# lisqzqng/Video-based-gait-analysis-for-dementia

Measured on AMD Instinct MI355X. Metric: frames/sec (224x224, seq=16), higher is better.
Workload: dtype f32

## Files before the change

video-based-gait-analysis-for-dementia_amd/csrc/grnet_run.cpp:

```cpp
#include "grnet_impl.h"

namespace grk { thread_local GraphRecorder* g_recorder = nullptr; }

int grnet::allocate() {
    if (plan_arena(compact, arena_plan)) return fail(GRNET_ESTATE, "the activation arena could not be planned: a launch group or the assignment violates the sharing rule");
    const size_t total = (size_t)arena_plan.total;
    arena_floats = total;
    void* q = nullptr;
    if (hipMalloc(&q, total * sizeof(float)) != hipSuccess)
        return fail(GRNET_ENOMEM, std::string("hipMalloc of the ") + (compact ? "compact " : "") + "activation arena (" + std::to_string(total * 4 >> 20) + " MiB) failed");
    arena = static_cast<float*>(q);
    if (hipMemset(arena, 0, 64 * sizeof(float)) != hipSuccess) return fail(GRNET_EHIP, "hipMemset failed");
    zeros = arena;
    if (hipEventCreateWithFlags(&ev_fork, hipEventDisableTiming) != hipSuccess) return fail(GRNET_EHIP, "hipEventCreate failed");
    if (int rc = install_schedule(max_frames)) return rc;
    if (hipStreamCreateWithFlags(&capture_stream, hipStreamNonBlocking) != hipSuccess) return fail(GRNET_EHIP, "hipStreamCreate failed");
    const size_t n = max_frames;
    int rc;
    if ((rc = dev_alloc(&d_plf, n * 128 * 24))) return rc;
    if ((rc = dev_alloc(&d_csf, n * 64 * 24))) return rc;
    if ((rc = dev_alloc(&d_stats, softmax_pool_ws_floats((int)n)))) return rc;
    if ((rc = dev_alloc(&d_rot6d, n * 144))) return rc;
    if ((rc = dev_alloc(&d_shape, n * 10))) return rc;
    if ((rc = dev_alloc(&d_cam, n * 3))) return rc;
// ... 291 lines not shown
    for (size_t oi = 0; oi < ops.size(); ++oi) {
        const Op& op = ops[oi];
        s = lane_stream[op.lane];
        const int lane = multi_lane ? op.lane : 0;
        if (lanes)
            for (int w : op.waits) HIP_TRY(hipStreamWaitEvent(s, op_events[w], 0));
        if (convs_only && op.kind != Op::CONV && op.kind != Op::FUSEUP) {
            if (lanes && op.record) HIP_TRY(hipEventRecord(op_events[oi], s));
            continue;
        }
        if (tl_start && !rec) HIP_TRY(hipEventRecord((*tl_start)[oi], s));
        if (rec) {
            rec->deps.clear();
            rec->n_chain = lane_last[lane] ? 1 : 0;
            if (lane_last[lane]) rec->deps.push_back(lane_last[lane]);
            if (multi_lane)
                for (int w : op.waits)
                    if (op_node[w] && std::find(rec->deps.begin(), rec->deps.end(), op_node[w]) == rec->deps.end()) rec->deps.push_back(op_node[w]);
        }
        static const char* abl_skip = GRNET_AB_STR(ABL_SKIP);
        if (abl_skip && (op.kind == Op::CONV || op.kind == Op::FUSEUP)) {
            const std::string lbl = op_label(op);
            bool skip = false;
            for (const char* q = abl_skip; *q;) {
                const char* e = strchr(q, ',');
                const std::string pat = e ? std::string(q, e) : std::string(q);
                if (!pat.empty() && lbl.find(pat) != std::string::npos) skip = true;
                q = e ? e + 1 : q + strlen(q);
            }
            if (skip) {
                if (tl_end && !rec) HIP_TRY(hipEventRecord((*tl_end)[oi], s));
                if (lanes && op.record) HIP_TRY(hipEventRecord(op_events[oi], s));
                continue;
            }
        }
        switch (op.kind) {
            case Op::CONVERT:
                HIP_TRY(launch_nchw_f32_to_nhwc_bf16(frames, base(v_in8), n, 3, 224, 224, 8, s));
                ++launches;
                break;
            case Op::CONV: {
                int nl = 1;
                if (int rc = launch_conv_op(convs[op.conv_idx], frames, n, s, &nl)) return rc;
                launches += nl;
                break;
            }
            case Op::SUM: {
                const auto& sv = sum_views[op.conv_idx];
                SumArgs a = op.sum;
                a.N = n;
                bind(sv.out, a.out, a.out_ctot, a.out_coff);
                for (int k = 0; k < a.n_add; ++k) {
                    bind(sv.adds[k].v, a.add[k], a.add_ctot[k], a.add_coff[k]);
                    a.add_shift[k] = sv.adds[k].shift;
                }
                if (dtype == 1) HIP_TRY(launch_fuse_sum_bf16(a, s));
                else HIP_TRY(launch_fuse_sum(a, s));
                ++launches;
                break;
            }
            case Op::FUSEUP:
                if (int rc = launch_fuse_up_op(fuse_ups[op.conv_idx], n, s)) return rc;
                ++launches;
                break;
            case Op::BILINEAR:
                if (dtype == 1) HIP_TRY(launch_bilinear2x_bf16(base(op.bin), base(op.bout), n, op.bin.c, op.bin.h, op.bin.w, s));
                else HIP_TRY(launch_bilinear2x(base(op.bin), base(op.bout), n, op.bin.c, op.bin.h, op.bin.w, s));
                ++launches;
                break;
            case Op::POOL:
                if (dtype == 1)
                    HIP_TRY(launch_softmax_pool_bf16(base(v_heat), v_heat.ctot, bf16_at(v_smpl_feats), 128, v_smpl_feats.ctot, bf16_at(v_csmap), 64,
                                                     v_csmap.ctot, d_stats, n, 56 * 56, s));
                else
                    HIP_TRY(launch_softmax_pool(base(v_heat), 25, base(v_smpl_feats), 128, base(v_csmap), 64, plf, csf, d_stats, n, 56 * 56, s));
                ++launches;
                break;
            case Op::TAIL:
                HIP_TRY(launch_head_tail(d_stats, true, plf, csf, tailw, rot6d, d_shape, d_cam, rotmat, theta, n, s));
                ++launches;
                break;
            case Op::SMPL:
                HIP_TRY(launch_smpl(d_shape, rotmat, d_cam, smpl, d_A, verts, kp3d, kp2d, n, s));
                launches += 4;
                break;
        }
        if (tl_end && !rec) HIP_TRY(hipEventRecord((*tl_end)[oi], s));
        if (lanes && op.record) HIP_TRY(hipEventRecord(op_events[oi], s));
        if (rec && !rec->deps.empty()) lane_last[lane] = op_node[oi] = rec->deps[0];
    }
    s = caller;
    if (lanes)
        for (int l = 1; l < lanes_used; ++l) {
            if (!join_lane[l]) continue;
            HIP_TRY(hipEventRecord(ev_join[l], side[l]));
            HIP_TRY(hipStreamWaitEvent(s, ev_join[l], 0));
        }
    if (!convs_only) {
        auto copy_out = [&](float* dst, const float* src, size_t bytes) -> int {
            if (!dst) return 0;
            if (!rec) { HIP_TRY(hipMemcpyAsync(dst, src, bytes, hipMemcpyDeviceToDevice, s)); return 0; }
            std::vector<hipGraphNode_t> deps;
            for (hipGraphNode_t nd : lane_last) if (nd) deps.push_back(nd);
            hipGraphNode_t node = nullptr;
            HIP_TRY(hipGraphAddMemcpyNode1D(&node, rec->graph, deps.data(), deps.size(), dst, src, bytes, hipMemcpyDeviceToDevice));
            return 0;
        };
        int rc;
        if (dtype == 1) {
            auto conv_out = [&](float* dst, const View& v) -> int {
                if (!dst) return 0;
                if (rec) {
                    rec->deps.clear();
                    for (hipGraphNode_t nd : lane_last) if (nd) rec->deps.push_back(nd);
                }
                HIP_TRY(launch_nhwc_bf16_to_nchw_f32(base(v), dst, n, v.c, v.h, v.w, v.ctot, v.coff, s));
                return 0;
            };
            if ((rc = conv_out(o.features, v_cat))) return rc;
            if ((rc = conv_out(o.part_attn, v_heat))) return rc;
            if ((rc = conv_out(o.smpl_feats, v_smpl_feats))) return rc;
        } else {
        if ((rc = copy_out(o.features, base(v_cat), (size_t)n * 480 * 3136 * 4))) return rc;
        if ((rc = copy_out(o.part_attn, base(v_heat), (size_t)n * 25 * 3136 * 4))) return rc;
        if ((rc = copy_out(o.smpl_feats, base(v_smpl_feats), (size_t)n * 128 * 3136 * 4))) return rc;
        }
        launches_last = launches;
    }
    return 0;
}

int grnet::head_from_feats(const float* plf, const float* csf, int n, const grnet_outputs_t& o, hipStream_t s) {
    const auto [rot6d, rotmat, theta, verts, kp3d, kp2d] = head_outputs(o);
    HIP_TRY(launch_head_tail_from_feats(plf, csf, tailw, rot6d, d_shape, d_cam, rotmat, theta, n, s));
    HIP_TRY(launch_smpl(d_shape, rotmat, d_cam, smpl, d_A, verts, kp3d, kp2d, n, s));
    if (o.point_local_feat && o.point_local_feat != plf) HIP_TRY(hipMemcpyAsync(o.point_local_feat, plf, (size_t)n * 3072 * 4, hipMemcpyDeviceToDevice, s));
    if (o.cam_shape_feats && o.cam_shape_feats != csf) HIP_TRY(hipMemcpyAsync(o.cam_shape_feats, csf, (size_t)n * 1536 * 4, hipMemcpyDeviceToDevice, s));
    return 0;
}

int grnet::gait_correct(const float* plf, const float* csf, const float* cam, int cam_ld, const float* bbox, const float* cimg, int b, int T,
                        const grnet_outputs_t& o, const grnet_gait_outputs_t& g, hipStream_t s) {
    if (int rc = gru_fault_check()) return rc;
    const size_t M = (size_t)b * T;
    const bool taps = taps_armed;
    if (taps) {
        size_t need = 0;
        if (featcorr_tap_floats(b, T, &need) != hipSuccess) { taps_armed = false; return fail(GRNET_EHIP, "device query for the tap layout failed"); }
        if (int rc = taps_begin(need + gru_tap_floats(b, T), "a gait-correction call")) return rc;
    }
    const size_t gru_need = gru_ws_floats(M, b);
    auto al = [](size_t f) { return (f + 63) & ~(size_t)63; };
    const size_t own = al(M * 3) + al((size_t)b * 3) + al(M * 4) + al(M * 3072);
    float* ws = nullptr;
    if (int rc = temporal_scratch(kGemmWsFloats + gru_need + featcorr_ws_floats(b, T) + own, &ws)) return rc;
    GemmWorkspaceLease lease(ws, kGemmWsFloats);
    float* p = ws + kGemmWsFloats;
    float* cparams = g.pred_cparam ? g.pred_cparam : p;   p += al(M * 3);
    float* avg = g.pred_avg ? g.pred_avg : p;             p += al((size_t)b * 3);
    float* phase = g.pred_phase ? g.pred_phase : p;       p += al(M * 4);
    float* new_plf = g.point_local_feat ? g.point_local_feat : p;   p += al(M * 3072);
    float* xc_buf = nullptr;
    const GruWorkspace w = gru_carve(p, M, b, &xc_buf);
    float* fws = p + gru_need;
    {
        TapLease tap_lease(taps ? &tap_sink : nullptr);
        HIP_TRY(launch_gait_cparams(cam, cam_ld, bbox, cimg, cparams, (int)M, s));
// ... 248 lines not shown
```

video-based-gait-analysis-for-dementia_amd/csrc/head_kernels.hip:

```cpp
#include "kernels.h"
#include "device.h"

namespace grk {

__global__ __launch_bounds__(256) void fuse_sum_kernel(const SumArgs a) {
    const int HW = a.H * a.W, n = blockIdx.x / a.C, c = blockIdx.x - n * a.C;
    const float inv_w = 1.0f / (float)a.W;
    for (int pix = threadIdx.x * 4; pix < HW; pix += 1024) {
        f32x4 v = f32x4{0.f, 0.f, 0.f, 0.f};
        for (int k = 0; k < a.n_add; ++k) {
            const int sh = a.add_shift[k];
            if (sh == 0) {
                v += *reinterpret_cast<const f32x4*>(a.add[k] + ((size_t)n * a.add_ctot[k] + a.add_coff[k] + c) * HW + pix);
            } else {
                const int hs = a.H >> sh, ws = a.W >> sh;
                const float* ap = a.add[k] + ((size_t)n * a.add_ctot[k] + a.add_coff[k] + c) * (hs * ws);
#pragma unroll
                for (int r = 0; r < 4; ++r) {
                    const int y = (int)(((float)(pix + r) + 0.5f) * inv_w), x = (pix + r) - y * a.W;
                    v[r] += ap[(y >> sh) * ws + (x >> sh)];
                }
            }
        }
        if (a.relu) {
// ... 398 lines not shown
            const f32x4 wv = *reinterpret_cast<const f32x4*>(wr + 4 * k), x = *reinterpret_cast<const f32x4*>(cs + 4 * k);
            acc += x * wv;
        }
        s_sp[o][seg] = (acc[0] + acc[1]) + (acc[2] + acc[3]);
    }
    __syncthreads();
    if (tid < 144) {
        const float acc = (s_pp[0][tid] + s_pp[1][tid]) + (s_pp[2][tid] + s_pp[3][tid]);
        s_pose[tid] = acc;
        rot6d[(size_t)n * 144 + tid] = acc;
    } else if (tid < 157) {
        const int o = tid - 144;
        float acc = 0.f;
#pragma unroll
        for (int seg = 0; seg < 8; ++seg) acc += s_sp[o][seg];
        s_sc[o] = acc + (o < 10 ? w.shape_b[o] : w.cam_b[o - 10]);
    }
    __syncthreads();
    if (tid < 24) {
        float R[9], aa[3];
        rot6d_to_rotmat_dev(&s_pose[tid * 6], R);
#pragma unroll
        for (int k = 0; k < 9; ++k) rotmat[(size_t)n * 216 + tid * 9 + k] = R[k];
        rotmat_to_aa_dev(R, aa);
        theta[(size_t)n * 85 + 3 + tid * 3 + 0] = aa[0];
        theta[(size_t)n * 85 + 3 + tid * 3 + 1] = aa[1];
        theta[(size_t)n * 85 + 3 + tid * 3 + 2] = aa[2];
    }
    if (tid >= 64 && tid < 74) {
        const int o = tid - 64;
        shape[(size_t)n * 10 + o] = s_sc[o];
        theta[(size_t)n * 85 + 75 + o] = s_sc[o];
    }
    if (tid >= 128 && tid < 131) {
        const int o = tid - 128;
        cam[(size_t)n * 3 + o] = s_sc[10 + o];
        theta[(size_t)n * 85 + o] = s_sc[10 + o];
    }
}

hipError_t launch_head_tail(const float* pool_ws, bool range_stats, float* plf, float* csf, TailWeights w, float* rot6d, float* shape, float* cam,
                            float* rotmat, float* theta, int N, hipStream_t s) {
    GRK_TRY(launch_k(head_tail_kernel<true>, dim3(N), dim3(256), 0, s, pool_ws + (size_t)N * kPoolStatsFloats, range_stats ? pool_ws : (const float*)nullptr, plf, csf,
                     w, rot6d, shape, cam, rotmat, theta));
    return hipGetLastError();
}

hipError_t launch_head_tail_from_feats(const float* plf, const float* csf, TailWeights w, float* rot6d, float* shape, float* cam, float* rotmat,
                                       float* theta, int N, hipStream_t s) {
    GRK_TRY(launch_k(head_tail_kernel<false>, dim3(N), dim3(256), 0, s, (const float*)nullptr, (const float*)nullptr, const_cast<float*>(plf), const_cast<float*>(csf), w,
                     rot6d, shape, cam, rotmat, theta));
    return hipGetLastError();
}

__global__ __launch_bounds__(256) void rot6d_to_rotmat_kernel(const float* __restrict__ x, float* __restrict__ R, int m) {
    const int i = blockIdx.x * 256 + threadIdx.x;
    if (i >= m) return;
    float xi[6], r[9];
#pragma unroll
    for (int k = 0; k < 6; ++k) xi[k] = x[(size_t)i * 6 + k];
    rot6d_to_rotmat_dev(xi, r);
#pragma unroll
    for (int k = 0; k < 9; ++k) R[(size_t)i * 9 + k] = r[k];
}
__global__ __launch_bounds__(256) void rotmat_to_aa_kernel(const float* __restrict__ R, float* __restrict__ aa, int m) {
    const int i = blockIdx.x * 256 + threadIdx.x;
    if (i >= m) return;
    float r[9], a[3];
#pragma unroll
    for (int k = 0; k < 9; ++k) r[k] = R[(size_t)i * 9 + k];
    rotmat_to_aa_dev(r, a);
#pragma unroll
    for (int k = 0; k < 3; ++k) aa[(size_t)i * 3 + k] = a[k];
}
hipError_t launch_rot6d_to_rotmat(const float* x, float* R, int m, hipStream_t s) {
    GRK_TRY(launch_k(rot6d_to_rotmat_kernel, dim3((m + 255) / 256), dim3(256), 0, s, x, R, m));
    return hipGetLastError();
}
hipError_t launch_rotmat_to_aa(const float* R, float* aa, int m, hipStream_t s) {
    GRK_TRY(launch_k(rotmat_to_aa_kernel, dim3((m + 255) / 256), dim3(256), 0, s, R, aa, m));
    return hipGetLastError();
}

__global__ __launch_bounds__(320) void smpl_chain_kernel(const float* __restrict__ betas, const float* __restrict__ rotmat, SmplTables t,
                                                           float* __restrict__ A_ws, float* __restrict__ kp3d, float* __restrict__ feat) {
    __shared__ float J[24][3];
    __shared__ float G[24][12];
    __shared__ float Rs[216];
    __shared__ int par[24], depth[24];
    const int n = blockIdx.x, tid = threadIdx.x;
    for (int e = tid; e < 216; e += 320) Rs[e] = rotmat[(size_t)n * 216 + e];
    if (tid < 24) par[tid] = t.parents[tid];
    for (int e = tid; e < 72; e += 320) {
        float v = t.J_template[e];
#pragma unroll
        for (int l = 0; l < 10; ++l) v += t.J_shapedirs[e * 10 + l] * betas[(size_t)n * 10 + l];
        J[e / 3][e % 3] = v;
    }
    for (int e = tid; e < kBlendK; e += 320) {
        float v = 0.f;
        if (e < 207) v = rotmat[(size_t)n * 216 + 9 + e] - ((e % 9 == 0 || e % 9 == 4 || e % 9 == 8) ? 1.f : 0.f);
        else if (e < 217) v = betas[(size_t)n * 10 + e - 207];
        else if (e == 217) v = 1.f;
        feat[(size_t)n * kBlendK + e] = v;
    }
    __syncthreads();
    if (tid < 24) {
        int d = 0;
        for (int p = par[tid]; p >= 0 && d < 24; p = par[p]) ++d;
        depth[tid] = d;
    }
    __syncthreads();
    const int ji = tid / 12, rc = tid - ji * 12, r = rc >> 2, c = rc & 3;
    const bool mine = tid < 288;
    const int myd = mine ? depth[ji] : -1, p = mine ? par[ji] : 0;
    for (int d = 0; d < 24; ++d) {
        if (mine && myd == d) {
            if (d == 0) {
                G[ji][rc] = c < 3 ? Rs[ji * 9 + r * 3 + c] : J[ji][r];
            } else {
                const float g0 = G[p][r * 4 + 0], g1 = G[p][r * 4 + 1], g2 = G[p][r * 4 + 2];
                if (c < 3) {
                    const float* Ri = Rs + ji * 9;
                    G[ji][rc] = g0 * Ri[c] + g1 * Ri[3 + c] + g2 * Ri[6 + c];
                } else {
                    const float t0 = J[ji][0] - J[p][0], t1 = J[ji][1] - J[p][1], t2 = J[ji][2] - J[p][2];
                    G[ji][rc] = g0 * t0 + g1 * t1 + g2 * t2 + G[p][r * 4 + 3];
                }
            }
        }
        __syncthreads();
        if (d >= 1 && __syncthreads_count(mine && myd > d) == 0) break;
    }
    for (int e = tid; e < 24 * 12; e += 320) {
        const int i = e / 12, rc2 = e % 12, r2 = rc2 / 4, c2 = rc2 % 4;
        float v = G[i][rc2];
        if (c2 == 3) {
            kp3d[((size_t)n * 29 + i) * 3 + r2] = v;
            v -= G[i][r2 * 4 + 0] * J[i][0] + G[i][r2 * 4 + 1] * J[i][1] + G[i][r2 * 4 + 2] * J[i][2];
        }
        A_ws[(size_t)n * 288 + e] = v;
    }
}

constexpr int kNumVerts = 6890;
constexpr int kBlendCols = kNumVerts * 3;

template <int MT>
__device__ __forceinline__ void blend_pass(const float* __restrict__ As, const float (&bv)[kBlendK / 4], float* __restrict__ Cs, int l15, int lq, int wave) {
    constexpr int LD = kBlendK + 1, KS = kBlendK / 4;
    f32x4 acc[MT];
#pragma unroll
    for (int m = 0; m < MT; ++m) acc[m] = f32x4{0.f, 0.f, 0.f, 0.f};
    const float* a0 = As + l15 * LD + lq;
#pragma unroll
    for (int ks = 0; ks < KS; ++ks)
#pragma unroll
        for (int m = 0; m < MT; ++m) acc[m] = __builtin_amdgcn_mfma_f32_16x16x4f32(a0[m * 16 * LD + 4 * ks], bv[ks], acc[m], 0, 0, 0);
#pragma unroll
    for (int m = 0; m < MT; ++m)
#pragma unroll
        for (int r = 0; r < 4; ++r) Cs[(m * 16 + lq * 4 + r) * 64 + wave * 16 + l15] = acc[m][r];
}

__global__ __launch_bounds__(256, 2) void smpl_blend_mfma_kernel(const float* __restrict__ feat, const float* __restrict__ blend, float* __restrict__ vposed,
                                                               int N) {
    constexpr int LD = kBlendK + 1, KS = kBlendK / 4;
    __shared__ float As[64 * LD];
    __shared__ __align__(16) float Cs[64 * 64];
    const int tid = threadIdx.x, lane = tid & 63, wave = tid >> 6, l15 = lane & 15, lq = lane >> 4;
    const int col = blockIdx.x * 64 + wave * 16 + l15;
    const bool cok = col < kBlendCols;
    const float* bp = blend + (cok ? col : 0) + (size_t)lq * kBlendCols;
    float bv[KS];
#pragma unroll
    for (int ks = 0; ks < KS; ++ks) bv[ks] = bp[(size_t)(4 * ks) * kBlendCols];
    for (int f0 = 0; f0 < N; f0 += 64) {
        const int nf = min(64, N - f0), mtiles = (nf + 15) >> 4;
        __syncthreads();
        {
            constexpr int UPR = kBlendK / 4, NU = (64 * UPR + 255) / 256;
            f32x4 v[NU];
#pragma unroll
            for (int i = 0; i < NU; ++i) {
                const int u = tid + 256 * i, f = u / UPR;
                v[i] = (u < mtiles * 16 * UPR && f < nf) ? *reinterpret_cast<const f32x4*>(feat + (size_t)(f0 + f) * kBlendK + 4 * (u - f * UPR))
                                                           : f32x4{0.f, 0.f, 0.f, 0.f};
            }
#pragma unroll
            for (int i = 0; i < NU; ++i) {
                const int u = tid + 256 * i, f = u / UPR, k = 4 * (u - f * UPR);
                if (u < mtiles * 16 * UPR) {
                    As[f * LD + k] = v[i][0]; As[f * LD + k + 1] = v[i][1]; As[f * LD + k + 2] = v[i][2]; As[f * LD + k + 3] = v[i][3];
                }
            }
        }
        __syncthreads();
        switch (mtiles) {
            case 1: blend_pass<1>(As, bv, Cs, l15, lq, wave); break;
            case 2: blend_pass<2>(As, bv, Cs, l15, lq, wave); break;
            case 3: blend_pass<3>(As, bv, Cs, l15, lq, wave); break;
            default: blend_pass<4>(As, bv, Cs, l15, lq, wave); break;
        }
        __syncthreads();
        const int cbase = blockIdx.x * 64;
#pragma unroll
        for (int i = 0; i < 8; ++i) {
            const int row = (tid >> 5) + 8 * i, c2 = (tid & 31) * 2;
            if (row < nf && cbase + c2 < kBlendCols)
                *reinterpret_cast<f32x2*>(vposed + (size_t)(f0 + row) * kBlendCols + cbase + c2) = *reinterpret_cast<const f32x2*>(Cs + row * 64 + c2);
        }
    }
}

__global__ __launch_bounds__(256) void smpl_skin_kernel(SmplTables t, const float* __restrict__ A_ws, float* __restrict__ verts) {
    __shared__ float sA[288];
    const int n = blockIdx.y, tid = threadIdx.x;
    for (int e = tid; e < 288; e += 256) sA[e] = A_ws[(size_t)n * 288 + e];
    __syncthreads();
    const int v = blockIdx.x * 256 + tid;
    if (v >= kNumVerts) return;
    float* pv = verts + ((size_t)n * kNumVerts + v) * 3;
    const float p0 = pv[0], p1 = pv[1], p2 = pv[2];
    float T[12];
#pragma unroll
    for (int e = 0; e < 12; ++e) T[e] = 0.f;
    for (int k = 0; k < t.skin_k; ++k) {
        const int j = t.skin_idx[(size_t)v * t.skin_k + k];
        const float wj = t.skin_w[(size_t)v * t.skin_k + k];
        if (j < 0) break;
#pragma unroll
        for (int e = 0; e < 12; ++e) T[e] += wj * sA[j * 12 + e];
    }
#pragma unroll
    for (int r = 0; r < 3; ++r) pv[r] = T[r * 4 + 0] * p0 + T[r * 4 + 1] * p1 + T[r * 4 + 2] * p2 + T[r * 4 + 3];
}

__global__ __launch_bounds__(256) void smpl_joints_kernel(const float* __restrict__ verts, const float* __restrict__ cam, SmplTables t,
                                                            float* __restrict__ kp3d, float* __restrict__ kp2d) {
    __shared__ float red[4][3];
    __shared__ float sj[29][3];
    const int n = blockIdx.x, tid = threadIdx.x, lane = tid & 63, wave = tid >> 6;
    const float* vn = verts + (size_t)n * kNumVerts * 3;
    float a0 = 0.f, a1 = 0.f, a2 = 0.f;
    for (int k = tid; k < t.thorax_n; k += 256) {
        const int v = t.thorax_idx[k];
        const float w = t.thorax_w[k];
        a0 += w * vn[v * 3]; a1 += w * vn[v * 3 + 1]; a2 += w * vn[v * 3 + 2];
    }
    a0 = wave_sum(a0); a1 = wave_sum(a1); a2 = wave_sum(a2);
    if (lane == 0) { red[wave][0] = a0; red[wave][1] = a1; red[wave][2] = a2; }
    if (tid < 72) sj[tid / 3][tid % 3] = kp3d[(size_t)n * 87 + tid];
    if (tid >= 96 && tid < 108) {
        const int e = tid - 96, jj = e / 3, d = e % 3;
        const int vid = jj == 0 ? 2746 : jj == 1 ? 2445 : jj == 2 ? 6191 : 5905;
        sj[24 + jj][d] = vn[vid * 3 + d];
    }
    __syncthreads();
    if (tid < 3) sj[28][tid] = red[0][tid] + red[1][tid] + red[2][tid] + red[3][tid];
    __syncthreads();
    if (tid < 87) kp3d[(size_t)n * 87 + tid] = sj[tid / 3][tid % 3];
    if (tid < 29 && cam != nullptr && kp2d != nullptr) {
        const float s = cam[(size_t)n * 3], tx = cam[(size_t)n * 3 + 1], ty = cam[(size_t)n * 3 + 2];
        const float tz = 2.f * 5000.f / (224.f * s + 1e-9f);
        const float X = sj[tid][0] + tx, Y = sj[tid][1] + ty, Z = sj[tid][2] + tz;
        kp2d[((size_t)n * 29 + tid) * 2 + 0] = 5000.f * (X / Z) / 112.f;
        kp2d[((size_t)n * 29 + tid) * 2 + 1] = 5000.f * (Y / Z) / 112.f;
    }
}

hipError_t launch_smpl(const float* betas, const float* rotmat, const float* cam, SmplTables t, float* A_ws, float* verts,
                       float* kp3d, float* kp2d, int N, hipStream_t s) {
    float* feat = A_ws + (size_t)N * 288;
    GRK_TRY(launch_k(smpl_chain_kernel, dim3(N), dim3(320), 0, s, betas, rotmat, t, A_ws, kp3d, feat));
    GRK_TRY(launch_k(smpl_blend_mfma_kernel, dim3((kBlendCols + 63) / 64), dim3(256), 0, s, (const float*)feat, t.blend, verts, N));
    GRK_TRY(launch_k(smpl_skin_kernel, dim3((kNumVerts + 255) / 256, N), dim3(256), 0, s, t, (const float*)A_ws, verts));
    GRK_TRY(launch_k(smpl_joints_kernel, dim3(N), dim3(256), 0, s, verts, cam, t, kp3d, kp2d));
    return hipGetLastError();
}

}
```

video-based-gait-analysis-for-dementia_amd/csrc/kernels.h:

```cpp
#pragma once
#include <hip/hip_runtime.h>
#include <stdint.h>
#include "raster_lines.h"
#include "seq_args.h"

#include <initializer_list>
#include <mutex>
#include <string>
#include <tuple>
#include <utility>
#include <vector>

#ifdef GRNET_ABLATION
#include <cstdlib>
#define GRNET_AB(name, dflt) (getenv("GRNET_" #name) ? atoi(getenv("GRNET_" #name)) : (dflt))
#define GRNET_AB_F(name, dflt) (getenv("GRNET_" #name) ? atof(getenv("GRNET_" #name)) : (dflt))
#define GRNET_AB_SET(name) (getenv("GRNET_" #name) != nullptr)
#define GRNET_AB_STR(name) getenv("GRNET_" #name)
#else
#define GRNET_AB(name, dflt) (dflt)
#define GRNET_AB_F(name, dflt) (dflt)
#define GRNET_AB_SET(name) false
#define GRNET_AB_STR(name) (static_cast<const char*>(nullptr))
#endif
// ... 113 lines not shown
    int pw_stream;
    int dbg;
    int prio;
    int blk0, wsplit;
};

hipError_t launch_conv(ConvArgs a, hipStream_t s, int tile_hint = 0);
struct ConvChoice { int family = 0, tps = 0, tcs = 0, nw = 0, waves = 0, width_variant = 0, rows = 0; };
hipError_t conv_choose(const ConvArgs& a, int tile_hint, ConvChoice* out);
int conv_pick_tc(int Cout);
hipError_t conv_init();
const char* conv_dominant_kernel_name();

bool conv_wino4_eligible(int cin, int cout, int ks, int stride, int h, int w, int n_add);
hipError_t launch_conv_wino4(ConvArgs a, hipStream_t s, int* n_launches = nullptr);
void pack_wino4_weights(const double* w_folded , int cout, int cin, int cin_pad, int cout_pad, float* out, int map_width = 56);
int conv_wino4_blocks(int cout, int map_width);
int conv_wino4_wide(int cout, int map_width);
struct Wino4Form { int waves = 0, nb = 0, npw = 0, gx = 0, gy = 0, xcd = 0, split = 0, full = 0, rest = 0; };
hipError_t conv_wino4_form(const ConvArgs& a, Wino4Form* f);

void wino4_transform_filter(const double* g33, double* u36);
bool conv_pw_eligible(int cin, int cout, int ks, int stride, int h, int w, int n_add);
hipError_t launch_conv_pw(ConvArgs a, hipStream_t s);
bool conv_stem_eligible(int cin, int cout, int ks, int stride, int h, int w, int n_add);
hipError_t launch_conv_stem(ConvArgs a, hipStream_t s);
void pack_stem_weights(const double* w_folded , float* out );
bool conv_wino4s_eligible(int cin, int cout, int ks, int stride, int h, int w, int n_add);
hipError_t launch_conv_wino4s(ConvArgs a, hipStream_t s, int ksplit);
int conv_wino4s_images_per_tile(int map_width);
int conv_wino4s_row_tiles(int map_width, int n_images, int* last_tile_images);
void pack_wino4r_weights(const double* w_folded , int cout, int cin, float* out );
struct SumArgs {
    float* out; int out_ctot, out_coff;
    int N, C, H, W, relu, n_add;
    const float* add[4]; int add_ctot[4], add_coff[4], add_shift[4];
};
hipError_t launch_fuse_sum(const SumArgs& a, hipStream_t s);

struct FuseUpSrc { const float* x; int ctot, coff; const float* w; };
struct FuseUpOut {
    float* out; int out_ctot, out_coff;
    const float* base; int base_ctot, base_coff;
    const float* bias;
    int relu, n_extra;
    const float* extra[2]; int extra_ctot[2], extra_coff[2];
    FuseUpSrc src[3];
};
struct FuseUpArgs { int N, nb; FuseUpOut o[3]; int only = -1; };
hipError_t launch_hr_fuse_up(const FuseUpArgs& a, hipStream_t s);
void pack_fuse_up_weights(const double* w_folded , int cout, int cin, float* out );
hipError_t launch_hr_fuse_up_bf16(const FuseUpArgs& a, hipStream_t s);
void pack_fuse_up_weights_bf16(const double* w_folded , int cout, int cin, unsigned short* out );

hipError_t launch_bilinear2x(const float* in, float* out, int N, int C, int H, int W, hipStream_t s);

hipError_t launch_crop_normalise(const unsigned char* img, int H, int W, int per_image, const float* bbox, float scale, int bgr,
                                 float* out, int N, hipStream_t s);

hipError_t launch_crop_normalise_cv(const unsigned char* img, int H, int W, int per_image, const double* maps, int mstride, int bgr, float* out, int N,
                                    hipStream_t s);

hipError_t launch_softmax_pool(const float* heat, int heat_ctot, const float* featA, int CA, const float* featB, int CB,
                               float* outA, float* outB, float* prob_ws, int N, int P, hipStream_t s);

struct TailWeights {
    const float* pose_w;
    const float* shape_w;
    const float* shape_b;
    const float* cam_w;
    const float* cam_b;
};
hipError_t launch_head_tail(const float* pool_ws, bool range_stats , float* plf, float* csf, TailWeights w, float* rot6d, float* shape, float* cam,
                            float* rotmat, float* theta, int N, hipStream_t s);
hipError_t launch_head_tail_from_feats(const float* plf, const float* csf, TailWeights w, float* rot6d, float* shape, float* cam, float* rotmat,
                                       float* theta, int N, hipStream_t s);
hipError_t launch_rot6d_to_rotmat(const float* x, float* R, int m, hipStream_t s);
hipError_t launch_rotmat_to_aa(const float* R, float* aa, int m, hipStream_t s);
size_t softmax_pool_ws_floats(int N);
constexpr int kPoolStatsFloats = 7 * 24 * 2;
constexpr int kPoolSplit = 7;

constexpr int kBlendK = 220;
constexpr int kSmplWsFloatsPerFrame = 288 + kBlendK;
struct SmplTables {
    const float* blend;
    const int* skin_idx;
    const float* skin_w;
    int skin_k;
    const float* J_template;
    const float* J_shapedirs;
    const float* lbs_weights;
    const int* thorax_idx;
    const float* thorax_w;
    int thorax_n;
    const int* parents;
    int extra_ptr[10];
    const int* extra_idx;
    const float* extra_w;
};
hipError_t launch_smpl(const float* betas, const float* rotmat, const float* cam, SmplTables t, float* A_ws,
                       float* verts, float* kp3d, float* kp2d, int N, hipStream_t s);

constexpr int kOneEuroBlock = 32;
struct OneEuroCoef { float a_d, one_minus_a_d, two_pi, min_cutoff, beta; };
hipError_t launch_one_euro(const float* x, int ld, int T, OneEuroCoef c, float* xhat, hipStream_t s);
hipError_t launch_aa_to_rotmat(const float* aa, float* R, int m, const float* betas0, float* betas_out, int nb, hipStream_t s);
int smooth_joint_count(int kind);
hipError_t launch_smpl_joints54(const float* kp29, const float* verts, SmplTables t, int kind, float* joints, int n, hipStream_t s);

constexpr int kBboxMaxJoints = 64;
constexpr int kBboxMaxFrames = 4096;
constexpr double kBboxMinPixel = 500., kBboxSmallScale = 1.8;
constexpr int kMedoidRows = 256;
constexpr int kMedoidTile = 1024;
constexpr int kMedoidMaxSplits = 64;
constexpr int kMedoidBatch = 128;
struct MedoidBatch { int n; int off[kMedoidBatch + 1]; };
__host__ __device__ inline int medoid_split_columns(int n, int splits) { return ((n + splits - 1) / splits + 7) & ~7; }
hipError_t launch_bbox_prepare(const double* joints, int K, int frames, double threshold, float* points, double* hgt, hipStream_t s);
hipError_t launch_medoid_rowsum(const float* points, const MedoidBatch& b, int splits, double* partial, hipStream_t s);
hipError_t launch_medoid_argmin(const float* points, const MedoidBatch& b, int seq0, int splits, const double* partial, int* index, double* cost,
                                float* centre, hipStream_t s);
hipError_t launch_bbox_assemble(const double* hgt, const MedoidBatch& b, int seq0, int K, const float* centre, double* bbox, hipStream_t s);

constexpr int kMetricMaxJoints = 64;
constexpr int kMetricBatch = 128;
struct MetricBatch { int n; int off[kMetricBatch + 1]; };
struct MetricJoints { int n_select, n_root; unsigned char select[kMetricMaxJoints], root[kMetricMaxJoints]; };
hipError_t launch_metric_joints(const float* pred, const float* gt, int J, int frames, const MetricJoints& mj, double unit, int has_verts, double* per_frame,
                                double* transform, hipStream_t s);
hipError_t launch_metric_accel(const float* pred, const float* gt, int J, const MetricBatch& b, const MetricJoints& mj, double unit, double* per_frame,
                               hipStream_t s);
hipError_t launch_metric_verts(const float* pred, const float* gt, int V, int frames, double unit, double* per_frame, hipStream_t s);
hipError_t launch_metric_seq_means(const double* per_frame, const MetricBatch& b, int seq0, int has_verts, double* seq_sum, long long* seq_cnt,
                                   double* per_seq, hipStream_t s);
hipError_t launch_metric_total(const double* seq_sum, const long long* seq_cnt, int n_seq, double* total, hipStream_t s);
hipError_t launch_procrustes(const double* K, int k, double* R, double* sigma, hipStream_t s);

constexpr int kTransMaxPairs = 64;
constexpr int kTransBatch = 64;
struct TransPairs { int n; int p3[kTransMaxPairs], p2[kTransMaxPairs]; };
struct TransBatch { int n; int off[kTransBatch + 1]; double cam[kTransBatch][3]; };
hipError_t launch_translation_fit(const float* joints3d, const float* joints2d, int K3, int K2, const TransPairs& pairs, const TransBatch& b, double threshold,
                                  int min_joints, double* per_frame, hipStream_t s);
hipError_t launch_translation_seq(const float* joints3d, int K3, int root, const TransBatch& b, int seq0, int fill, double* per_frame, double* per_seq,
                                  hipStream_t s);

constexpr int kTrackMaxJoints = 64;
constexpr int kTrackMaxKernel = 31;
constexpr double kTrackMaxSigma = 16.;
constexpr int kTrackMaxRadius = 64;
constexpr int kTrackMaxSeqs = 8192;
constexpr int kTrackThreads = 1024;
constexpr int kTrackLdsFrames = 1024;
hipError_t launch_track_frames(const double* joints, int K, int frames, double vis_thresh, double* params, unsigned long long* words, hipStream_t s);
hipError_t launch_track_sequences(const int* off, int n_seq, const double* weights, int radius, int ksize, int pad, const double* params,
                                  const unsigned long long* words, double* work, double* boxes, int* status, int* range, hipStream_t s);
hipError_t launch_track_filter(const int* off, int n_seq, const double* x, const double* weights, int radius, int ksize, int pad, double* out, hipStream_t s);
hipError_t launch_seq_gauss_columns(const int* off, int n_seq, int channels, const double* weights, int radius, int frames, const double* raw, double* out,
                                    int cols, int col0, hipStream_t s);

constexpr int kGaitMaxWindow = 32;
constexpr int kGaitThreads = 256;
constexpr int kGaitLdsWords = 64;
struct GaitTable { int j[8]; };
inline size_t gait_mask_words(int frames, int n_seq) { return (size_t)(frames >> 6) + (size_t)n_seq + 1; }
// ... 231 lines not shown
```

Baseline: 4572.

## Fuse SMPL pipeline into two kernels: blend+chain and skin+joints

The four SMPL launches become two. The kinematic chain now runs as extra blocks inside the blend kernel, reusing its LDS, and the blend kernel stages its features directly from rotmat and betas instead of reading a feat buffer. Skinning and joint regression are merged, with the joint blocks recomputing the skinned thorax and extra vertices from vposed rather than reading finished verts. This removes two launches and the inter-kernel dependencies, at the cost of redundant skinning work in the joint block and a larger per-frame workspace.

```diff
diff --git a/video-based-gait-analysis-for-dementia_amd/csrc/grnet_run.cpp b/video-based-gait-analysis-for-dementia_amd/csrc/grnet_run.cpp
--- a/video-based-gait-analysis-for-dementia_amd/csrc/grnet_run.cpp
+++ b/video-based-gait-analysis-for-dementia_amd/csrc/grnet_run.cpp
@@ -397,7 +397,7 @@
                 break;
             case Op::SMPL:
                 HIP_TRY(launch_smpl(d_shape, rotmat, d_cam, smpl, d_A, verts, kp3d, kp2d, n, s));
-                launches += 4;
+                launches += 2;
                 break;
         }
         if (tl_end && !rec) HIP_TRY(hipEventRecord((*tl_end)[oi], s));
diff --git a/video-based-gait-analysis-for-dementia_amd/csrc/head_kernels.hip b/video-based-gait-analysis-for-dementia_amd/csrc/head_kernels.hip
--- a/video-based-gait-analysis-for-dementia_amd/csrc/head_kernels.hip
+++ b/video-based-gait-analysis-for-dementia_amd/csrc/head_kernels.hip
@@ -504,69 +504,76 @@
     return hipGetLastError();
 }
 
-__global__ __launch_bounds__(320) void smpl_chain_kernel(const float* __restrict__ betas, const float* __restrict__ rotmat, SmplTables t,
-                                                           float* __restrict__ A_ws, float* __restrict__ kp3d, float* __restrict__ feat) {
-    __shared__ float J[24][3];
-    __shared__ float G[24][12];
-    __shared__ float Rs[216];
-    __shared__ int par[24], depth[24];
-    const int n = blockIdx.x, tid = threadIdx.x;
-    for (int e = tid; e < 216; e += 320) Rs[e] = rotmat[(size_t)n * 216 + e];
-    if (tid < 24) par[tid] = t.parents[tid];
-    for (int e = tid; e < 72; e += 320) {
-        float v = t.J_template[e];
-#pragma unroll
-        for (int l = 0; l < 10; ++l) v += t.J_shapedirs[e * 10 + l] * betas[(size_t)n * 10 + l];
-        J[e / 3][e % 3] = v;
-    }
-    for (int e = tid; e < kBlendK; e += 320) {
-        float v = 0.f;
-        if (e < 207) v = rotmat[(size_t)n * 216 + 9 + e] - ((e % 9 == 0 || e % 9 == 4 || e % 9 == 8) ? 1.f : 0.f);
-        else if (e < 217) v = betas[(size_t)n * 10 + e - 207];
-        else if (e == 217) v = 1.f;
-        feat[(size_t)n * kBlendK + e] = v;
+constexpr int kNumVerts = 6890;
+constexpr int kBlendCols = kNumVerts * 3;
+constexpr int kBlendBlocks = (kBlendCols + 63) / 64;
+constexpr int kSkinBlocks = (kNumVerts + 255) / 256;
+
+__device__ __forceinline__ float dot3_r(float a0, float b0, float a1, float b1, float a2, float b2) {
+#pragma clang fp contract(off)
+    return __builtin_fmaf(a0, b0, a1 * b1) + a2 * b2;
+}
+
+struct ChainLds {
+    float J[24][3];
+    float G[24][12];
+    float Rs[216];
+    int par[24], depth[24];
+};
+
+__device__ __forceinline__ void chain_entry(ChainLds& L, int d, int ji, int p, int rc) {
+    const int r = rc >> 2, c = rc & 3;
+    if (d == 0) {
+        L.G[ji][rc] = c < 3 ? L.Rs[ji * 9 + r * 3 + c] : L.J[ji][r];
+    } else {
+        const float g0 = L.G[p][r * 4 + 0], g1 = L.G[p][r * 4 + 1], g2 = L.G[p][r * 4 + 2];
+        if (c < 3) {
+            const float* Ri = L.Rs + ji * 9;
+            L.G[ji][rc] = dot3_r(g0, Ri[c], g1, Ri[3 + c], g2, Ri[6 + c]);
+        } else {
+            const float t0 = L.J[ji][0] - L.J[p][0], t1 = L.J[ji][1] - L.J[p][1], t2 = L.J[ji][2] - L.J[p][2];
+            L.G[ji][rc] = dot3_r(g0, t0, g1, t1, g2, t2) + L.G[p][r * 4 + 3];
+        }
+    }
+}
+
+__device__ __forceinline__ void smpl_chain_role(ChainLds& L, int n, int tid, const float* __restrict__ betas, const float* __restrict__ rotmat,
+                                                const SmplTables& t, float* __restrict__ A_ws, float* __restrict__ kp3d) {
+    if (tid < 216) L.Rs[tid] = rotmat[(size_t)n * 216 + tid];
+    if (tid < 24) L.par[tid] = t.parents[tid];
+    if (tid < 72) {
+#pragma clang fp contract(off)
+        float v = t.J_template[tid];
+#pragma unroll
+        for (int l = 0; l < 10; ++l) v += t.J_shapedirs[tid * 10 + l] * betas[(size_t)n * 10 + l];
+        L.J[tid / 3][tid % 3] = v;
     }
     __syncthreads();
     if (tid < 24) {
         int d = 0;
-        for (int p = par[tid]; p >= 0 && d < 24; p = par[p]) ++d;
-        depth[tid] = d;
-    }
-    __syncthreads();
-    const int ji = tid / 12, rc = tid - ji * 12, r = rc >> 2, c = rc & 3;
-    const bool mine = tid < 288;
-    const int myd = mine ? depth[ji] : -1, p = mine ? par[ji] : 0;
+        for (int p = L.par[tid]; p >= 0 && d < 24; p = L.par[p]) ++d;
+        L.depth[tid] = d;
+    }
+    __syncthreads();
+    const int ji0 = tid / 12, rc0 = tid - ji0 * 12, ji1 = (256 + tid) / 12, rc1 = 256 + tid - ji1 * 12;
+    const bool two = tid < 32;
+    const int d0 = L.depth[ji0], p0 = L.par[ji0], d1 = two ? L.depth[ji1] : -1, p1 = two ? L.par[ji1] : 0;
     for (int d = 0; d < 24; ++d) {
-        if (mine && myd == d) {
-            if (d == 0) {
-                G[ji][rc] = c < 3 ? Rs[ji * 9 + r * 3 + c] : J[ji][r];
-            } else {
-                const float g0 = G[p][r * 4 + 0], g1 = G[p][r * 4 + 1], g2 = G[p][r * 4 + 2];
-                if (c < 3) {
-                    const float* Ri = Rs + ji * 9;
-                    G[ji][rc] = g0 * Ri[c] + g1 * Ri[3 + c] + g2 * Ri[6 + c];
-                } else {
-                    const float t0 = J[ji][0] - J[p][0], t1 = J[ji][1] - J[p][1], t2 = J[ji][2] - J[p][2];
-                    G[ji][rc] = g0 * t0 + g1 * t1 + g2 * t2 + G[p][r * 4 + 3];
-                }
-            }
-        }
+        if (d0 == d) chain_entry(L, d, ji0, p0, rc0);
+        if (d1 == d) chain_entry(L, d, ji1, p1, rc1);
         __syncthreads();
-        if (d >= 1 && __syncthreads_count(mine && myd > d) == 0) break;
-    }
-    for (int e = tid; e < 24 * 12; e += 320) {
+        if (d >= 1 && __syncthreads_count(d0 > d || d1 > d) == 0) break;
+    }
+    for (int e = tid; e < 24 * 12; e += 256) {
         const int i = e / 12, rc2 = e % 12, r2 = rc2 / 4, c2 = rc2 % 4;
-        float v = G[i][rc2];
+        float v = L.G[i][rc2];
         if (c2 == 3) {
             kp3d[((size_t)n * 29 + i) * 3 + r2] = v;
-            v -= G[i][r2 * 4 + 0] * J[i][0] + G[i][r2 * 4 + 1] * J[i][1] + G[i][r2 * 4 + 2] * J[i][2];
+            v -= dot3_r(L.G[i][r2 * 4 + 0], L.J[i][0], L.G[i][r2 * 4 + 1], L.J[i][1], L.G[i][r2 * 4 + 2], L.J[i][2]);
         }
         A_ws[(size_t)n * 288 + e] = v;
     }
 }
-
-constexpr int kNumVerts = 6890;
-constexpr int kBlendCols = kNumVerts * 3;
 
 template <int MT>
 __device__ __forceinline__ void blend_pass(const float* __restrict__ As, const float (&bv)[kBlendK / 4], float* __restrict__ Cs, int l15, int lq, int wave) {
@@ -585,38 +592,46 @@
         for (int r = 0; r < 4; ++r) Cs[(m * 16 + lq * 4 + r) * 64 + wave * 16 + l15] = acc[m][r];
 }
 
-__global__ __launch_bounds__(256, 2) void smpl_blend_mfma_kernel(const float* __restrict__ feat, const float* __restrict__ blend, float* __restrict__ vposed,
-                                                               int N) {
+__device__ __forceinline__ void stage_rows(float* __restrict__ As, const float* __restrict__ rotmat, const float* __restrict__ betas, int f0, int nf,
+                                           int m, int e) {
+    constexpr int LD = kBlendK + 1;
+    if (e >= kBlendK) return;
+    const bool rot = e < 207;
+    const float one = (rot && (e % 9 == 0 || e % 9 == 4 || e % 9 == 8)) ? 1.f : 0.f;
+    const float* src = rot ? rotmat + 9 + e : betas + (min(e, 216) - 207);
+    const size_t stride = rot ? 216 : 10;
+    float x[16];
+#pragma unroll
+    for (int i = 0; i < 16; ++i) x[i] = src[(size_t)(f0 + min(m * 16 + i, nf - 1)) * stride];
+#pragma unroll
+    for (int i = 0; i < 16; ++i) {
+        const float v = rot ? x[i] - one : e < 217 ? x[i] : e == 217 ? 1.f : 0.f;
+        As[(m * 16 + i) * LD + e] = m * 16 + i < nf ? v : 0.f;
+    }
+}
+
+__global__ __launch_bounds__(256, 2) void smpl_blend_chain_kernel(const float* __restrict__ betas, const float* __restrict__ rotmat, SmplTables t,
+                                                                  float* __restrict__ A_ws, float* __restrict__ kp3d, float* __restrict__ vposed, int N) {
     constexpr int LD = kBlendK + 1, KS = kBlendK / 4;
     __shared__ float As[64 * LD];
     __shared__ __align__(16) float Cs[64 * 64];
+    static_assert(sizeof(ChainLds) <= sizeof(float) * 64 * LD, "the chain role's LDS lies in As");
     const int tid = threadIdx.x, lane = tid & 63, wave = tid >> 6, l15 = lane & 15, lq = lane >> 4;
+    if (blockIdx.x >= kBlendBlocks) {
+        smpl_chain_role(*reinterpret_cast<ChainLds*>(As), blockIdx.x - kBlendBlocks, tid, betas, rotmat, t, A_ws, kp3d);
+        return;
+    }
     const int col = blockIdx.x * 64 + wave * 16 + l15;
     const bool cok = col < kBlendCols;
-    const float* bp = blend + (cok ? col : 0) + (size_t)lq * kBlendCols;
+    const float* bp = t.blend + (cok ? col : 0) + (size_t)lq * kBlendCols;
     float bv[KS];
 #pragma unroll
     for (int ks = 0; ks < KS; ++ks) bv[ks] = bp[(size_t)(4 * ks) * kBlendCols];
     for (int f0 = 0; f0 < N; f0 += 64) {
         const int nf = min(64, N - f0), mtiles = (nf + 15) >> 4;
         __syncthreads();
-        {
-            constexpr int UPR = kBlendK / 4, NU = (64 * UPR + 255) / 256;
-            f32x4 v[NU];
-#pragma unroll
-            for (int i = 0; i < NU; ++i) {
-                const int u = tid + 256 * i, f = u / UPR;
-                v[i] = (u < mtiles * 16 * UPR && f < nf) ? *reinterpret_cast<const f32x4*>(feat + (size_t)(f0 + f) * kBlendK + 4 * (u - f * UPR))
-                                                           : f32x4{0.f, 0.f, 0.f, 0.f};
-            }
-#pragma unroll
-            for (int i = 0; i < NU; ++i) {
-                const int u = tid + 256 * i, f = u / UPR, k = 4 * (u - f * UPR);
-                if (u < mtiles * 16 * UPR) {
-                    As[f * LD + k] = v[i][0]; As[f * LD + k + 1] = v[i][1]; As[f * LD + k + 2] = v[i][2]; As[f * LD + k + 3] = v[i][3];
-                }
-            }
-        }
+        stage_rows(As, rotmat, betas, f0, nf, 0, tid);
+        for (int m = 1; m < mtiles; ++m) stage_rows(As, rotmat, betas, f0, nf, m, tid);
         __syncthreads();
         switch (mtiles) {
             case 1: blend_pass<1>(As, bv, Cs, l15, lq, wave); break;
@@ -635,15 +650,8 @@
     }
 }
 
-__global__ __launch_bounds__(256) void smpl_skin_kernel(SmplTables t, const float* __restrict__ A_ws, float* __restrict__ verts) {
-    __shared__ float sA[288];
-    const int n = blockIdx.y, tid = threadIdx.x;
-    for (int e = tid; e < 288; e += 256) sA[e] = A_ws[(size_t)n * 288 + e];
-    __syncthreads();
-    const int v = blockIdx.x * 256 + tid;
-    if (v >= kNumVerts) return;
-    float* pv = verts + ((size_t)n * kNumVerts + v) * 3;
-    const float p0 = pv[0], p1 = pv[1], p2 = pv[2];
+__device__ __forceinline__ void skin_vertex(const SmplTables& t, const float* __restrict__ sA, const float* __restrict__ vp, int v, float (&out)[3]) {
+    const float p0 = vp[v * 3], p1 = vp[v * 3 + 1], p2 = vp[v * 3 + 2];
     float T[12];
 #pragma unroll
     for (int e = 0; e < 12; ++e) T[e] = 0.f;
@@ -652,31 +660,45 @@
         const float wj = t.skin_w[(size_t)v * t.skin_k + k];
         if (j < 0) break;
 #pragma unroll
-        for (int e = 0; e < 12; ++e) T[e] += wj * sA[j * 12 + e];
-    }
-#pragma unroll
-    for (int r = 0; r < 3; ++r) pv[r] = T[r * 4 + 0] * p0 + T[r * 4 + 1] * p1 + T[r * 4 + 2] * p2 + T[r * 4 + 3];
-}
-
-__global__ __launch_bounds__(256) void smpl_joints_kernel(const float* __restrict__ verts, const float* __restrict__ cam, SmplTables t,
-                                                            float* __restrict__ kp3d, float* __restrict__ kp2d) {
+        for (int e = 0; e < 12; ++e) T[e] = __builtin_fmaf(wj, sA[j * 12 + e], T[e]);
+    }
+    out[0] = T[3] + __builtin_fmaf(p2, T[2], __builtin_fmaf(p1, T[1], p0 * T[0]));
+    out[1] = T[7] + __builtin_fmaf(p2, T[6], __builtin_fmaf(p0, T[4], p1 * T[5]));
+    out[2] = T[11] + __builtin_fmaf(p2, T[10], __builtin_fmaf(p0, T[8], p1 * T[9]));
+}
+
+__global__ __launch_bounds__(256) void smpl_skin_joints_kernel(SmplTables t, const float* __restrict__ A_ws, const float* __restrict__ vposed,
+                                                                 const float* __restrict__ cam, float* __restrict__ verts, float* __restrict__ kp3d,
+                                                                 float* __restrict__ kp2d) {
+    __shared__ float sA[288];
     __shared__ float red[4][3];
     __shared__ float sj[29][3];
-    const int n = blockIdx.x, tid = threadIdx.x, lane = tid & 63, wave = tid >> 6;
-    const float* vn = verts + (size_t)n * kNumVerts * 3;
+    const int n = blockIdx.y, tid = threadIdx.x, lane = tid & 63, wave = tid >> 6;
+    for (int e = tid; e < 288; e += 256) sA[e] = A_ws[(size_t)n * 288 + e];
+    __syncthreads();
+    const float* vp = vposed + (size_t)n * kBlendCols;
+    float x[3];
+    if (blockIdx.x < kSkinBlocks) {
+        const int v = blockIdx.x * 256 + tid;
+        if (v >= kNumVerts) return;
+        skin_vertex(t, sA, vp, v, x);
+        float* pv = verts + ((size_t)n * kNumVerts + v) * 3;
+        pv[0] = x[0]; pv[1] = x[1]; pv[2] = x[2];
+        return;
+    }
     float a0 = 0.f, a1 = 0.f, a2 = 0.f;
     for (int k = tid; k < t.thorax_n; k += 256) {
-        const int v = t.thorax_idx[k];
         const float w = t.thorax_w[k];
-        a0 += w * vn[v * 3]; a1 += w * vn[v * 3 + 1]; a2 += w * vn[v * 3 + 2];
+        skin_vertex(t, sA, vp, t.thorax_idx[k], x);
+        a0 = __builtin_fmaf(w, x[0], a0); a1 = __builtin_fmaf(w, x[1], a1); a2 = __builtin_fmaf(w, x[2], a2);
     }
     a0 = wave_sum(a0); a1 = wave_sum(a1); a2 = wave_sum(a2);
     if (lane == 0) { red[wave][0] = a0; red[wave][1] = a1; red[wave][2] = a2; }
     if (tid < 72) sj[tid / 3][tid % 3] = kp3d[(size_t)n * 87 + tid];
     if (tid >= 96 && tid < 108) {
         const int e = tid - 96, jj = e / 3, d = e % 3;
-        const int vid = jj == 0 ? 2746 : jj == 1 ? 2445 : jj == 2 ? 6191 : 5905;
-        sj[24 + jj][d] = vn[vid * 3 + d];
+        skin_vertex(t, sA, vp, jj == 0 ? 2746 : jj == 1 ? 2445 : jj == 2 ? 6191 : 5905, x);
+        sj[24 + jj][d] = d == 0 ? x[0] : d == 1 ? x[1] : x[2];
     }
     __syncthreads();
     if (tid < 3) sj[28][tid] = red[0][tid] + red[1][tid] + red[2][tid] + red[3][tid];
@@ -684,7 +706,7 @@
     if (tid < 87) kp3d[(size_t)n * 87 + tid] = sj[tid / 3][tid % 3];
     if (tid < 29 && cam != nullptr && kp2d != nullptr) {
         const float s = cam[(size_t)n * 3], tx = cam[(size_t)n * 3 + 1], ty = cam[(size_t)n * 3 + 2];
-        const float tz = 2.f * 5000.f / (224.f * s + 1e-9f);
+        const float tz = 2.f * 5000.f / __builtin_fmaf(224.f, s, 1e-9f);
         const float X = sj[tid][0] + tx, Y = sj[tid][1] + ty, Z = sj[tid][2] + tz;
         kp2d[((size_t)n * 29 + tid) * 2 + 0] = 5000.f * (X / Z) / 112.f;
         kp2d[((size_t)n * 29 + tid) * 2 + 1] = 5000.f * (Y / Z) / 112.f;
@@ -693,11 +715,9 @@
 
 hipError_t launch_smpl(const float* betas, const float* rotmat, const float* cam, SmplTables t, float* A_ws, float* verts,
                        float* kp3d, float* kp2d, int N, hipStream_t s) {
-    float* feat = A_ws + (size_t)N * 288;
-    GRK_TRY(launch_k(smpl_chain_kernel, dim3(N), dim3(320), 0, s, betas, rotmat, t, A_ws, kp3d, feat));
-    GRK_TRY(launch_k(smpl_blend_mfma_kernel, dim3((kBlendCols + 63) / 64), dim3(256), 0, s, (const float*)feat, t.blend, verts, N));
-    GRK_TRY(launch_k(smpl_skin_kernel, dim3((kNumVerts + 255) / 256, N), dim3(256), 0, s, t, (const float*)A_ws, verts));
-    GRK_TRY(launch_k(smpl_joints_kernel, dim3(N), dim3(256), 0, s, verts, cam, t, kp3d, kp2d));
+    float* vposed = A_ws + (size_t)N * 288;
+    GRK_TRY(launch_k(smpl_blend_chain_kernel, dim3(kBlendBlocks + N), dim3(256), 0, s, betas, rotmat, t, A_ws, kp3d, vposed, N));
+    GRK_TRY(launch_k(smpl_skin_joints_kernel, dim3(kSkinBlocks + 1, N), dim3(256), 0, s, t, (const float*)A_ws, (const float*)vposed, cam, verts, kp3d, kp2d));
     return hipGetLastError();
 }
 
diff --git a/video-based-gait-analysis-for-dementia_amd/csrc/kernels.h b/video-based-gait-analysis-for-dementia_amd/csrc/kernels.h
--- a/video-based-gait-analysis-for-dementia_amd/csrc/kernels.h
+++ b/video-based-gait-analysis-for-dementia_amd/csrc/kernels.h
@@ -219,7 +219,7 @@
 constexpr int kPoolSplit = 7;
 
 constexpr int kBlendK = 220;
-constexpr int kSmplWsFloatsPerFrame = 288 + kBlendK;
+constexpr int kSmplWsFloatsPerFrame = 288 + 6890 * 3;
 struct SmplTables {
     const float* blend;
     const int* skin_idx;
```

After: 4600 (median of 6 runs). No clear change (+0.6%).
